# Traneptora/jxlatte

Measured on AMD Instinct MI355X. Metric: Mpixels/s decoded (VarDCT 4K frame) at 1/2/4/8 MI355X vs host-CPU jxlatte, higher is better.
Workload: dtype f32; 1 GPU; vardct4k: 8 independent 3840x2160 VarDCT frames per GPU (mix=default, Gab + EPF x2 + XYB, f32 out), inputs resident in HBM; frames_per_gpu=8, frames_total=8, frame_seeds=1000 + i, frame i on rank i mod 1, distinct_frames=8, streams=2, kernel_launches_per_frame=2

## Files before the change

jxlatte_amd/csrc/host.hip:

```cpp
#include "jxl_internal.h"
#include "modular_tend.h"
#include "pfm_check.h"
#include "varblock_check.h"
#include "palette_check.h"
#include "modchain_check.h"
#include "palette_ops.h"

#include <algorithm>
#include <chrono>
#include <cmath>
#include <cstdarg>
#include <cstdio>
#include <cstring>
#include <cstdlib>
#include <string>
#include <atomic>
#include <thread>
#include <vector>
#include <mutex>
#include <limits>

using namespace jxl;
namespace jxl {
thread_local hipEvent_t g_restore_kernel_ev[2] = {nullptr, nullptr};
// ... 172 lines not shown
    std::vector<std::pair<const jxl_ctx*, uint64_t>> batch_key;
    struct BatchLaunch { int cls, n_frames, grid_x; size_t lds_bytes, offset; };
    DevBuf batch_wg3_args;
    void* h_map16 = nullptr;
    bool map16_nofill = false;
    bool is_feeder = false;
    hipEvent_t map16_ev = nullptr;
    bool map16_inflight = false;
    hipEvent_t out_ev = nullptr;
    bool out_inflight = false;
    size_t h_map16_bytes = 0;
    bool map16_valid = false;
    DevBuf stage16;
    static constexpr int kGrpSlots = 8;
    void* h_grp = nullptr;
    const void* h_grp_dev = nullptr;
    hipEvent_t grp_ev[kGrpSlots] = {};
    bool grp_inflight[kGrpSlots] = {};
    int grp_slot = 0;
    std::vector<uint8_t> grp_written;
    uint32_t* h_sp = nullptr;
    const void* h_sp_dev = nullptr;
    size_t sp_alloc_words = 0, sp_map_words = 0;
    bool sp_valid = false;
    hipEvent_t sp_ev = nullptr;
    bool sp_inflight = false;
    SparseRec* h_sp_tab = nullptr;
    const SparseRec* h_sp_tab_dev = nullptr;
    size_t sp_tab_cap = 0, sp_tab_used = 0;
    DevBuf sp_rej;
    bool sp_rej_live = false;
    std::vector<float> h_weights_in;
    int32_t h_woffs_in[51] = {};
    DevBuf wg3_items[2];
    int wg3_item_count[2] = {0, 0};
    std::vector<BatchLaunch> batch_launches;
    hipEvent_t batch_ev = nullptr;
    bool timing = false;
    static constexpr int kEvSlots = 32;
    hipEvent_t ev[kEvSlots][3] = {};
    hipEvent_t kev[kEvSlots][2] = {};
    bool kev_valid = false;
    int ev_runs = 0;
    bool owns_stream = true;
    PlanePool* pool = nullptr;
    size_t pool_set_bytes = 0;
    size_t priv_a_bytes = 0;
    static constexpr int kAux = 12;
    int n_aux = 1;
    hipStream_t aux[kAux] = {};
    hipEvent_t fork_ev = nullptr, join_ev[kAux] = {};

    std::vector<DevBuf> mod_bufs;
    std::vector<ModOp> mod_ops;
    std::vector<ModOp> mod_ops_fused;
    std::vector<ModChan> mod_out;
    bool mod_ran = false;
    DevBuf mod_flag;
    int32_t* mod_flag_host = nullptr;
    hipEvent_t mod_ev = nullptr, mod_join = nullptr;
    bool mod_pending = false;
    int mod_redos = 0;
    int mod_launches = 0;
    std::vector<PalRun> mod_pal_runs;
    DevBuf mod_pal_count;
    unsigned int* mod_pal_count_host = nullptr;
// ... 587 lines not shown
            if (!c->hfm_sub[ch].ensure(4 * std::max<size_t>(1, h_hfm_sub[ch].size()))) return fail(c, JXL_ERR_OOM, "device allocation failed");
            HIP_TRY(c, hipMemcpyAsync(c->hfm_sub[ch].p, h_hfm_sub[ch].data(), 4 * h_hfm_sub[ch].size(), hipMemcpyHostToDevice, c->stream));
        }
        HIP_TRY(c, hipStreamSynchronize(c->stream));
    }
    const size_t nc = (size_t)c->bh * c->bw, nt = (size_t)c->th * c->tw;
    std::vector<int> wg3_tab[2];
    for (int k = 0; k < 2; k++) {
        c->wg3_item_count[k] = 0;
        for (const auto& tl : c->type_launches) {
            if (tl.cls != 2 + k) continue;
            wg3_item_table(c->h_blocks.data(), c->bw, tl.segs.data(), (int)tl.segs.size(), k, c->woffs, wg3_tab[k], wg3_grid_cap(k == 1));
            c->wg3_item_count[k] = (int)(wg3_tab[k].size() / 8);
        }
    }
    mark("item tables");
    tab_wait(c);
    {
        const volatile float cf = (float)c->p.color_factor;
        for (size_t i = 0; i < nt; i++) {
            const volatile float qx = (float)c->h_xfy[i] / cf, qb = (float)c->h_bfy[i] / cf;
            c->h_kx[i] = c->p.base_corr_x + qx;
            c->h_kb[i] = c->p.base_corr_b + qb;
        }
    }
    build_inv_sigma(c->h_hf_mul.data(), c->h_sharp.data(), nc, c->p.global_scale_f, c->p.epf_sharp_lut, c->h_isig.data());
    wg3_build_tables(c->p.quant_bias, c->p.quant_bias_numerator, c->p.scale_factor, reinterpret_cast<float*>(c->h_tab + c->off_dq));
    mark("CfL factors, inverse sigma, dequantisation tables");
    size_t o = c->tab_fixed;
    const size_t off_blocks = o, n_blk = sizeof(DevBlock) * c->h_blocks.size();
    o = tab_up(o + std::max<size_t>(16, n_blk));
    const size_t off_items = o, n_items = sizeof(WorkItem) * items.size();
    o = tab_up(o + std::max<size_t>(16, n_items));
    size_t off_wg3[2];
    for (int k = 0; k < 2; k++) {
        off_wg3[k] = o;
        o = tab_up(o + std::max<size_t>(16, sizeof(int) * wg3_tab[k].size()));
    }
    const size_t total = o;
    if (!tab_reserve(c, total, c->tab_fixed)) return fail(c, JXL_ERR_OOM, "host allocation failed (table staging)");
    tab_bind_fixed(c, nc, nt);
    if (n_blk) memcpy(c->h_tab + off_blocks, c->h_blocks.data(), n_blk);
    if (n_items) memcpy(c->h_tab + off_items, items.data(), n_items);
    for (int k = 0; k < 2; k++) {
        if (!wg3_tab[k].empty()) memcpy(c->h_tab + off_wg3[k], wg3_tab[k].data(), sizeof(int) * wg3_tab[k].size());
    }
    if (total > c->tab.cap || !c->tab.p) {
        HIP_TRY(c, hipStreamSynchronize(c->stream));
        if (!c->tab.ensure(total + total / 4)) return fail(c, JXL_ERR_OOM, "device allocation failed (frame tables)");
    }
    mark("staging");
    if (!c->tab_ev) HIP_TRY(c, hipEventCreateWithFlags(&c->tab_ev, hipEventDisableTiming));
    static const bool tab_zero = !(getenv("JXL_TABLE_ZEROCOPY") && atoi(getenv("JXL_TABLE_ZEROCOPY")) == 0);
    if (!(tab_zero && c->h_tab_pinned && copy_zero(c, c->tab.p, c->h_tab, total, false, 64, false) == 1))
        HIP_TRY(c, hipMemcpyAsync(c->tab.p, c->h_tab, total, hipMemcpyHostToDevice, c->stream));
    HIP_TRY(c, hipEventRecord(c->tab_ev, c->stream));
    c->tab_inflight = true;
    {
        char* d = static_cast<char*>(c->tab.p);
        c->hf_mul.view(d + c->off_hfm, 4 * nc);
        c->sharp.view(d + c->off_sharp, 4 * nc);
        c->xfy.view(d + c->off_kx, 4 * nt);
        c->bfy.view(d + c->off_kb, 4 * nt);
        for (int i = 0; i < 3; i++) c->lf[i].view(d + c->off_lf[i], 4 * nc);
        c->inv_sigma_tab.view(d + c->off_isig, 4 * nc);
        c->dq_tab.view(d + c->off_dq, 4 * (size_t)kWg3DqTabFloats);
        c->blocks.view(d + off_blocks, std::max<size_t>(16, n_blk));
        c->items.view(d + off_items, std::max<size_t>(16, n_items));
        for (int k = 0; k < 2; k++) c->wg3_items[k].view(d + off_wg3[k], sizeof(int) * wg3_tab[k].size());
    }
    for (const auto& job : c->lf_jobs) {
        const jxl_lfquant_desc& d = job.d;
        if (c->sub) {
            for (int ch = 0; ch < 3; ch++) {
                const int h2 = d.cells_h >> c->sy[ch], w2 = d.cells_w >> c->sx[ch], bw2 = c->bw >> c->sx[ch];
                const size_t n2 = (size_t)h2 * w2;
                if (!c->lfq_tmp[ch].ensure(4 * std::max<size_t>(1, n2))) return fail(c, JXL_ERR_OOM, "device allocation failed (LF image)");
                HIP_TRY(c, hipMemcpyAsync(c->lfq_tmp[ch].p, job.q[ch].data(), 4 * n2, hipMemcpyHostToDevice, c->stream));
                launch_lf_dequant_plain(c->lfq_tmp[ch].as<int32_t>(), c->lf[ch].as<float>(), h2, w2,
                                        (int64_t)((d.lfg_y * 256) >> c->sy[ch]) * bw2 + ((d.lfg_x * 256) >> c->sx[ch]), bw2,
                                        d.scaled_dequant[ch], d.extra_precision, c->stream);
            }
            HIP_TRY(c, hipStreamSynchronize(c->stream));
            continue;
        }
        const size_t n = (size_t)d.cells_h * d.cells_w;
        const int32_t* dq[3];
        for (int ch = 0; ch < 3; ch++) {
            if (!c->lfq_tmp[ch].ensure(4 * std::max<size_t>(1, n))) return fail(c, JXL_ERR_OOM, "device allocation failed (LF image)");
            HIP_TRY(c, hipMemcpyAsync(c->lfq_tmp[ch].p, job.q[ch].data(), 4 * n, hipMemcpyHostToDevice, c->stream));
            dq[ch] = c->lfq_tmp[ch].as<int32_t>();
        }
        float* lfp[3] = {c->lf[0].as<float>(), c->lf[1].as<float>(), c->lf[2].as<float>()};
        launch_lf_dequant(dq, lfp, d.cells_h, d.cells_w, (int64_t)(d.lfg_y * 256) * c->bw + d.lfg_x * 256, c->bw, d.scaled_dequant,
                          d.extra_precision, c->p.base_corr_x, c->p.base_corr_b, c->p.color_factor, d.x_factor_lf, d.b_factor_lf,
                          d.adaptive_smoothing, c->stream);
        HIP_TRY(c, hipStreamSynchronize(c->stream));
    }
    c->llf_alias = c->large_count == 0;
    if (!c->llf_alias)
        for (int ch = 0; ch < 3; ch++)
// ... 164 lines not shown

__global__ void k_clock_probe(unsigned long long ticks, unsigned long long* out) {
    const unsigned long long r0 = __builtin_amdgcn_s_memrealtime(), c0 = __builtin_amdgcn_s_memtime();
    unsigned long long r1 = r0;
    while (r1 - r0 < ticks) {
        __builtin_amdgcn_s_sleep(8);
        r1 = __builtin_amdgcn_s_memrealtime();
    }
    const unsigned long long c1 = __builtin_amdgcn_s_memtime();
    if (threadIdx.x == 0) {
        out[0] = c1 - c0;
        out[1] = r1 - r0;
    }
}
extern "C" int jxl_debug_wg3_item_table(const int32_t* types, const int32_t* n_blocks, int n_types, int frame_bw, int grid, int32_t* out, int cap) {
    std::vector<DevBlock> blocks;
    std::vector<IdctSegment> segs;
    int cell = 0;
    for (int k = 0; k < n_types; k++) {
        const int t = types[k];
        if (t < 0 || t >= JXL_NUM_TRANSFORM_TYPES || n_blocks[k] <= 0) return -1;
        segs.push_back(IdctSegment{t, (int)blocks.size(), n_blocks[k]});
        const int cw = JXL_TT[t].pw / 8, chh = JXL_TT[t].ph / 8;
        for (int i = 0; i < n_blocks[k]; i++, cell += cw * chh)
            blocks.push_back(DevBlock{(uint16_t)((cell / std::max(1, frame_bw)) & 0xffff), (uint16_t)(cell % std::max(1, frame_bw)), (uint32_t)t, 0u, 1});
    }
    int32_t woffs[3 * 17] = {};
    std::vector<int> tab;
    wg3_item_table(blocks.data(), frame_bw, segs.data(), (int)segs.size(), 0, woffs, tab, grid);
    const int n = (int)(tab.size() / 8);
    if (n > cap) return -1;
    std::copy(tab.begin(), tab.end(), out);
    return n;
}
extern "C" int64_t jxl_debug_intermediate_bytes(int device) {
    return device >= 0 && device < 64 ? (int64_t)g_inter_bytes[device].load(std::memory_order_relaxed) : -1;
}
extern "C" int jxl_debug_set_plane_a_tiled(int on) { return g_plane_a_tiled.exchange(on ? 1 : 0, std::memory_order_relaxed); }
extern "C" int jxl_debug_last_plane_a_tiled(const jxl_ctx* c) { return c ? c->last_plane_a_tiled : 0; }
extern "C" int jxl_debug_set_palette_fuse(int on) { return g_palette_fuse.exchange(on ? 1 : 0, std::memory_order_relaxed); }
extern "C" int jxl_debug_last_palette_run(const jxl_ctx* c, int32_t out[3]) {
    if (!c || !out) return -1;
    for (int i = 0; i < 3; i++) out[i] = c->mod_pal_stats[i];
    return 0;
}
extern "C" int jxl_debug_last_restore_launches(const jxl_ctx* c, int32_t codes[2]) {
    if (!c) return 0;
    for (int i = 0; i < 2 && codes; i++) codes[i] = i < c->last_restore_n ? c->last_restore_code[i] : 0;
    return c->last_restore_n;
}
extern "C" void jxl_debug_build_inv_sigma(const int32_t* hf_mul, const int32_t* sharpness, int64_t n, float global_scale_f,
                                          const float sharp_lut[8], float* out) {
    if (hf_mul && sharpness && sharp_lut && out && n > 0) build_inv_sigma(hf_mul, sharpness, (size_t)n, global_scale_f, sharp_lut, out);
}
extern "C" void jxl_debug_wg3_tables(const float quant_bias[3], float quant_bias_numerator, const float scale_factor[3], float* out) {
    if (quant_bias && scale_factor && out) wg3_build_tables(quant_bias, quant_bias_numerator, scale_factor, out);
}
extern "C" int64_t jxl_debug_read_inv_sigma(jxl_ctx* c, float* out, int64_t cap) {
    if (!c || !out || bind(c) != JXL_OK || !c->frame_open) return -1;
    const int64_t nc = (int64_t)c->bh * c->bw;
    if (cap < nc || finalize_tables(c) != JXL_OK || !c->inv_sigma_tab.p) return -1;
    if (hipStreamSynchronize(c->stream) != hipSuccess || hipMemcpy(out, c->inv_sigma_tab.p, 4 * (size_t)nc, hipMemcpyDeviceToHost) != hipSuccess) return -1;
    return nc;
}
extern "C" int jxl_debug_last_palette(const jxl_ctx* c, int64_t* delta_pixels) {
    if (!c) return 0;
// ... 211 lines not shown
    if (c->spl_ev) (void)hipEventDestroy(c->spl_ev);
    if (c->h_spl) {
        if (c->h_spl_pinned) (void)hipHostFree(c->h_spl);
        else free(c->h_spl);
    }
    for (auto& b : c->mod_bufs) b.release();
    for (int i = 0; i < jxl_ctx::kEvSlots; i++)
        for (int j = 0; j < 3; j++)
            if (c->ev[i][j]) (void)hipEventDestroy(c->ev[i][j]);
    for (int i = 0; i < jxl_ctx::kEvSlots; i++)
        for (int j = 0; j < 2; j++)
            if (c->kev[i][j]) (void)hipEventDestroy(c->kev[i][j]);
    if (c->fork_ev) (void)hipEventDestroy(c->fork_ev);
    if (c->batch_ev) (void)hipEventDestroy(c->batch_ev);
    c->batch_wg3_args.release();
    c->mod_flag.release();
    if (c->mod_flag_host) (void)hipHostFree(c->mod_flag_host);
    c->mod_flag_host = nullptr;
    c->mod_pal_count.release();
    if (c->mod_pal_count_host) (void)hipHostFree(c->mod_pal_count_host);
    c->mod_pal_count_host = nullptr;
    if (c->mod_ev) (void)hipEventDestroy(c->mod_ev);
    if (c->mod_join) (void)hipEventDestroy(c->mod_join);
    c->mod_ev = c->mod_join = nullptr;
    c->stage16.release();
    if (c->map16_ev) (void)hipEventDestroy(c->map16_ev);
    if (c->out_ev) (void)hipEventDestroy(c->out_ev);
    if (c->h_map16) (void)hipHostFree(c->h_map16);
    c->h_map16 = nullptr;
    if (c->sp_ev) (void)hipEventDestroy(c->sp_ev);
    if (c->h_sp) (void)hipHostFree(c->h_sp);
    if (c->h_sp_tab) (void)hipHostFree(c->h_sp_tab);
    c->sp_rej.release();
    c->wg3_items[0].release();
    c->wg3_items[1].release();
    c->batch_restore_args.release();
    for (int i = 0; i < jxl_ctx::kAux; i++) {
        if (c->aux[i]) { (void)hipStreamSynchronize(c->aux[i]); (void)hipStreamDestroy(c->aux[i]); }
        if (c->join_ev[i]) (void)hipEventDestroy(c->join_ev[i]);
    }
    if (c->stream && c->owns_stream) (void)hipStreamDestroy(c->stream);
    delete c;
}

jxl_status jxl_ctx_synchronize(jxl_ctx* c) {
    jxl_status st = bind(c);
    if (st) return st;
    HIP_TRY(c, hipStreamSynchronize(c->stream));
    return JXL_OK;
}

void* jxl_ctx_stream(jxl_ctx* c) { return c ? (void*)c->stream : nullptr; }

jxl_status jxl_ctx_set_stream(jxl_ctx* c, void* stream) {
    jxl_status st = bind(c);
    if (st) return st;
    HIP_TRY(c, hipStreamSynchronize(c->stream));
    pool_detach(c);
    if (c->owns_stream && c->stream) (void)hipStreamDestroy(c->stream);
    c->stream = (hipStream_t)stream;
    c->owns_stream = false;
    (void)pool_of(c);
    return JXL_OK;
}

jxl_status jxl_vardct_begin_frame(jxl_ctx* c, const jxl_vardct_params* p) {
// ... 798 lines not shown
    int launches = 0;
    float* B[3] = {c->planeB[0].as<float>(), c->planeB[1].as<float>(), c->planeB[2].as<float>()};
    hipEvent_t* evs = c->ev[c->ev_runs % jxl_ctx::kEvSlots];
    if (c->timing) (void)hipEventRecord(evs[0], s);
    if ((p.stages & JXL_STAGE_IDCT) && !idct_done) {
        DevFrame f;
        fill_dev_frame(c, f);
        const DevBlock* blocks = c->blocks.as<DevBlock>();
        const WorkItem* items = c->items.as<WorkItem>();
        if (c->llf_count > 0) {
            float* L[3] = {c->llf[0].as<float>(), c->llf[1].as<float>(), c->llf[2].as<float>()};
            launch_llf(f, blocks, c->llf_first, c->llf_count, L, s);
            launches++;
        }
        auto frame_of = [&](int channel) {
            DevFrame fc = f;
            if (channel >= 0) {
                fc.no_cfl = 1;
                fc.width = c->W >> c->sx[channel];
                fc.height = c->H >> c->sy[channel];
                fc.bw = c->bw >> c->sx[channel];
                fc.bh = c->bh >> c->sy[channel];
                fc.hf_mul = c->hfm_sub[channel].as<int32_t>();
            }
            return fc;
        };
        static const int wg3_grid = wg3_grid_cap(false);
        static const int wg3_grid_big = wg3_grid_cap(true);
        Wg3Args wa[2];
        int wn[2] = {0, 0};
        for (const auto& tl : c->type_launches)
            if (tl.cls >= 2) {
                const int k = tl.cls - 2;
                wn[k] = build_wg3_args(f, blocks, tl.segs.data(), (int)tl.segs.size(), k, A, wa[k], tiled);
                if (wn[k] < 0) return fail(c, JXL_ERR_STATE, "IDCT launch: too many segments");
                if (c->wg3_item_count[k] < wn[k]) return fail(c, JXL_ERR_STATE, "IDCT launch: item list out of date");
                if (wn[k] > 0) wa[k].total_items = wn[k] = c->wg3_item_count[k];
                wa[k].items = c->wg3_items[k].as<int>();
            }
        const int n_k = (int)c->type_launches.size() + (int)c->special_launches.size();
        const bool fork = n_k > 1 && c->n_aux > 0;
        if (wn[0] > 0 || wn[1] > 0) {
            hipStream_t side = fork ? c->aux[0] : s;
            if (fork) {
                (void)hipEventRecord(c->fork_ev, s);
                (void)hipStreamWaitEvent(side, c->fork_ev, 0);
            }
            if (wn[1] > 0) {
                launch_idct_wg3(wa[1], true, wg3_grid_big, side);
                launches++;
            }
            if (wn[0] > 0) {
                launch_idct_wg3(wa[0], false, wg3_grid, s);
                launches++;
            }
            if (fork) {
                (void)hipEventRecord(c->join_ev[0], side);
                (void)hipStreamWaitEvent(s, c->join_ev[0], 0);
            }
        } else {
            int used = 0;
            if (fork) {
                (void)hipEventRecord(c->fork_ev, s);
                used = std::min(n_k - 1, c->n_aux);
                for (int i = 0; i < used; i++) (void)hipStreamWaitEvent(c->aux[i], c->fork_ev, 0);
            }
            int k = 0;
// ... 182 lines not shown
        if (!c->frame_open) return fail(c, JXL_ERR_STATE, "begin_frame first");
        st = finalize_tables(c);
        if (st) return st;
        if (!ensure_private_planes(c, 4 * (size_t)c->W * c->H)) return fail(c, JXL_ERR_OOM, "device allocation failed for a %dx%d frame", c->W, c->H);
        if ((st = pre_run_zero(c))) return st;
        ok = batchable(c);
    }
    if (!ok) {
        for (int i = 0; i < n; i++) {
            const jxl_status st = run_frame(ctxs[i], false);
            if (st) return st;
        }
        return JXL_OK;
    }
    bool same = (int)c0->batch_key.size() == n;
    for (int i = 0; i < n && same; i++) same = c0->batch_key[i].first == ctxs[i] && c0->batch_key[i].second == ctxs[i]->tables_gen;
    if (!same) {
        c0->batch_launches.clear();
        std::vector<Wg3Args> wg3_args;
        for (int cls : {11, 12}) {
            const int which = cls - 11;
            jxl_ctx::BatchLaunch bl{cls, 0, 0, 0, wg3_args.size() * sizeof(Wg3Args)};
            int max_n = 0;
            for (int i = 0; i < n; i++) {
                jxl_ctx* c = ctxs[i];
                DevFrame f;
                fill_dev_frame(c, f);
                float* A[3] = {c->planeA[0].as<float>(), c->planeA[1].as<float>(), c->planeA[2].as<float>()};
                const jxl_ctx::TypeLaunch* tl = nullptr;
                for (const auto& t : c->type_launches)
                    if (t.cls == which + 2) tl = &t;
                if (!tl) continue;
                Wg3Args a;
                const int items = build_wg3_args(f, c->blocks.as<DevBlock>(), tl->segs.data(), (int)tl->segs.size(), which, A, a);
                if (items < 0) return fail(c0, JXL_ERR_STATE, "IDCT launch: too many segments");
                if (items <= 0) continue;
                if (c->wg3_item_count[which] < items) return fail(c0, JXL_ERR_STATE, "IDCT launch: item list out of date");
                a.total_items = c->wg3_item_count[which];
                a.items = c->wg3_items[which].as<int>();
                max_n = std::max(max_n, items);
                bl.lds_bytes = std::max(bl.lds_bytes, wg3_lds_bytes(a));
                wg3_args.push_back(a);
                bl.n_frames++;
            }
            if (bl.n_frames <= 0) continue;
            const int cap = wg3_grid_cap(which == 1);
            bl.grid_x = std::min(max_n, std::max(1, (cap + bl.n_frames - 1) / bl.n_frames));
            c0->batch_launches.push_back(bl);
        }
        HIP_TRY(c0, hipSetDevice(c0->device));
        if (!c0->batch_wg3_args.ensure(std::max<size_t>(sizeof(Wg3Args), wg3_args.size() * sizeof(Wg3Args))))
            return fail(c0, JXL_ERR_OOM, "device allocation failed (batch arguments)");
        HIP_TRY(c0, hipStreamSynchronize(c0->stream));
        if (c0->n_aux > 0) HIP_TRY(c0, hipStreamSynchronize(c0->aux[0]));
        if (!wg3_args.empty())
            HIP_TRY(c0, hipMemcpy(c0->batch_wg3_args.p, wg3_args.data(), wg3_args.size() * sizeof(Wg3Args), hipMemcpyHostToDevice));
        c0->batch_key.clear();
        for (int i = 0; i < n; i++) c0->batch_key.emplace_back(ctxs[i], ctxs[i]->tables_gen);
        c0->batch_restore_valid = false;
        if (!c0->batch_ev) HIP_TRY(c0, hipEventCreateWithFlags(&c0->batch_ev, hipEventDisableTiming));
    }
    hipStream_t s0 = c0->stream;
    for (int i = 1; i < n; i++) {
        (void)hipEventRecord(ctxs[i]->fork_ev, ctxs[i]->stream);
        (void)hipStreamWaitEvent(s0, ctxs[i]->fork_ev, 0);
    }
    const bool fork = c0->n_aux > 0 && c0->batch_launches.size() > 1;
// ... 2294 lines not shown
```

jxlatte_amd/csrc/jxl_internal.h:

```cpp
#pragma once
#include <hip/hip_runtime.h>
#include <vector>
#include <cmath>
#include <stdint.h>
#include "../../include/jxlatte_amd.h"
#include "../../include/jxl_transform_types.h"
#include "plane_tiled.h"
#include "blend_ops.h"
#include "patch_compile.h"
#include "modchain_check.h"

namespace jxl {

constexpr int kLutTotal = 86870;

struct DevBlock {
    uint16_t cy, cx;
    uint32_t type;
    uint32_t cfl_zero;
    int32_t hf_mul;
};

static_assert(sizeof(DevBlock) == 16, "one dwordx4 per block record");

struct WorkItem {
    uint32_t type;
    uint32_t first;
    uint32_t count;
};

struct DevFrame {
    int32_t no_cfl;
    int32_t width, height;
    int32_t bw, bh;
    int32_t tw, th;
    const int32_t* coeff[3];
    const float* lf[3];
    const float* llf[3];
    const int32_t* hf_mul;
    const int32_t* sharpness;
// ... 20 lines not shown
    for (int j = 0; j < l; j++) o += ((1 << j) - 1) << j;
    return o;
}

struct EpfParams {
    float channel_scale[3];
    float sigma_scale;
    float border_sad_mul;
    float inv_sigma_modular;
};

struct XybParams {
    float sm[9];
    float ob[3];
    float cob[3];
};

struct MultiArgs {
    static constexpr int kMaxSeg = 12;
    DevFrame f;
    const DevBlock* blocks;
    const WorkItem* items;
    int n_seg;
    int seg_b0[kMaxSeg + 1];
    int seg_n[kMaxSeg];
    int seg_type[kMaxSeg];
    int seg_first[kMaxSeg];
    int seg_nblocks[kMaxSeg];
    int nch, ch0;
    float *o0, *o1, *o2;
};
struct IdctSegment { int type, first_block, n_blocks; };

struct Wg3Seg { int type, first_block, n_blocks, item_base; };
struct Wg3Args {
    static constexpr int kMaxSeg = 21;
    DevFrame f;
    const DevBlock* blocks;
    float *o0, *o1, *o2;
    int n_seg, total_items;
    int img_floats;
    int llf_in_item;
    const int* items;
    Wg3Seg seg[kMaxSeg];
    int tiled;
};

constexpr int kWg3DqTabFloats = 3 * 128 + 3 * 256;
void wg3_build_tables(const float quant_bias[3], float quant_bias_numerator, const float scale_factor[3], float* out );
void wg3_item_table(const DevBlock* host_blocks, int frame_bw, const IdctSegment* segs, int n_seg, int which, const int32_t* woffs,
                    std::vector<int>& out, int grid);
int wg3_grid_cap(bool big);
bool wg3_handles(int type);
bool wg3_big(int type);
int build_wg3_args(const DevFrame& f, const DevBlock* blocks, const IdctSegment* segs, int n_seg, int which, float* const out[3],
                   Wg3Args& a, bool tiled = false);
void launch_idct_wg3(const Wg3Args& a, bool big, int grid_cap, hipStream_t s);
size_t wg3_lds_bytes(const Wg3Args& a);
void launch_idct_wg3_batch(const Wg3Args* dev_args, int n_frames, bool big, int grid_x, size_t lds, hipStream_t s);


int idct_class_of(int type);
void launch_idct_multi(const DevFrame& f, const DevBlock* blocks, int cls, const IdctSegment* segs, int n_seg, int ch,
                       float* const out[3], hipStream_t s);
void launch_idct_special(const DevFrame& f, const DevBlock* blocks, const WorkItem* items, int n_items, float* const out[3], hipStream_t s);
int medium_blocks_per_wg(int type);
void launch_llf(const DevFrame& f, const DevBlock* blocks, int first, int count, float* const llf[3], hipStream_t s);
void launch_idct_large(const DevFrame& f, const DevBlock* blocks, const DevBlock* host_blocks, int first, int count,
                       float* const out[3], float* const scratch[3], hipStream_t s, int* n_launches);
void launch_accumulate(int32_t* dst, const int32_t* src, int64_t n, hipStream_t s);

struct SparseRec {
    uint32_t chunk_first;
    uint32_t chunk_src;
    uint32_t count_wide;
    uint32_t where;
};
static_assert(sizeof(SparseRec) == 16, "one dwordx4 per run record");
constexpr int kSparseMaxRuns = 2048;
struct SparseGeom {
    int32_t* plane[3];
    int32_t W, H;
    int32_t sx[3], sy[3];
};
struct SparseRect { int32_t W, y0, x0, gw, gh; };
__host__ __device__ inline SparseRect sparse_rect(int W, int H, int sx, int sy, int group) {
    const int grs = (W + 255) >> 8, gy = group / grs, gx = group - gy * grs;
    const int gh = H - gy * 256 < 256 ? H - gy * 256 : 256, gw = W - gx * 256 < 256 ? W - gx * 256 : 256;
    return SparseRect{W >> sx, (gy * 256) >> sy, (gx * 256) >> sx, gw >> sx, gh >> sy};
// ... 372 lines not shown
```

jxlatte_amd/csrc/k_idct_wg3.hip:

```cpp
#include "jxl_internal.h"
#include <cstdio>
#include <cstdlib>
#include <algorithm>
#include <vector>
#include "../../include/jxl_tables.h"

namespace jxl {

#include "idct_small.h"

namespace {

#ifndef JXL_WG3_SCALAR_MAC
typedef float v2f __attribute__((ext_vector_type(2)));
__device__ __forceinline__ v2f lut_pair(const __attribute__((address_space(4))) float* lr, int j) {
    return ((const __attribute__((address_space(4))) v2f*)lr)[j];
}
#else
struct v2f {
    float x, y;
};
__device__ __forceinline__ v2f operator*(v2f a, v2f b) { return v2f{a.x * b.x, a.y * b.y}; }
__device__ __forceinline__ v2f operator+(v2f a, v2f b) { return v2f{a.x + b.x, a.y + b.y}; }
__device__ __forceinline__ v2f operator-(v2f a, v2f b) { return v2f{a.x - b.x, a.y - b.y}; }
// ... 306 lines not shown

template <int P>
__device__ __forceinline__ Item item_of(const Wg3Args& a, int& gi, int step) {
    Item it{-1, 0, 0, 0u, 0};
    while (gi < a.total_items) {
        const auto* w = (const __attribute__((address_space(4))) int*)a.items + 8 * gi;
        const int type = w[0];
        if (type != -2) {
            it.type = type;
            it.first = w[1];
            it.nb = w[2];
            it.geo = (uint32_t)w[3];
            it.gi = gi;
            break;
        }
        gi += step;
    }
    return it;
}

__device__ __forceinline__ int llf_lane_block(int tid, int lgA) { return (int)(((uint32_t)tid * 0xAAABu) >> 17) >> lgA; }

template <int NG, int WS>
struct Raw {
    v4i q[NG][3];
    v4f w[WS][3];
    float kx[NG], kb[NG];
    float hfm[NG];
    float llf;
    int rowx;
    uint32_t ok;
};

template <int NG>
struct Recs {
    int gx[NG], gz[NG], gw[NG];
    int lx;
};

template <int T, int NG>
__device__ __forceinline__ void load_recs(const Wg3Args& a, const Item& it, int tid, Recs<NG>& rc) {
    const int lgGPB = (int)((it.geo >> 4) & 15u), lgA = (int)((it.geo >> 8) & 7u);
#pragma unroll
    for (int j = 0; j < NG; j++) {
        rc.gx[j] = rc.gz[j] = 0;
        rc.gw[j] = 1;
        const int b = (tid + T * j) >> lgGPB;
        if (it.type >= 0 && b < it.nb) {
            const auto* w = (const __attribute__((address_space(4))) int*)a.blocks + 4 * (it.first + b);
            rc.gx[j] = w[0];
            rc.gz[j] = w[2];
            rc.gw[j] = w[3];
        }
    }
    rc.lx = 0;
    const int bl = llf_lane_block(tid, lgA);
    if (it.type >= 0 && bl < it.nb) rc.lx = ((const __attribute__((address_space(4))) int*)a.blocks)[4 * (it.first + bl)];
}

template <typename P>
__device__ __forceinline__ const __attribute__((address_space(1))) P* sgpr_ptr(const P* p) {
    unsigned long long u = (unsigned long long)p;
    asm volatile("" : "+s"(u));
    return (const __attribute__((address_space(1))) P*)u;
}

template <int T, int NG, int WS>
__device__ __forceinline__ void prefetch(const Wg3Args& a, const Item& it, int tid, const Recs<NG>& rc, Raw<NG, WS>& raw) {
    const DevFrame& f = a.f;
    raw.ok = 0;
    raw.llf = 0.0f;
    const int lgW4 = (int)(it.geo & 7u), lgGPB = (int)((it.geo >> 4) & 15u);
    const float* wtab = ((it.geo >> 15) & 1u) ? f.weights_t : f.weights;
    const auto* irec = (const __attribute__((address_space(4))) int*)a.items + 8 * it.gi;
    const float* wt[3] = {wtab + irec[4], wtab + irec[5], wtab + irec[6]};
    const __attribute__((address_space(1))) int32_t* cp[3] = {sgpr_ptr(f.coeff[0]), sgpr_ptr(f.coeff[1]), sgpr_ptr(f.coeff[2])};
    const auto* kxt = sgpr_ptr(f.kx_tab);
    const auto* kbt = sgpr_ptr(f.kb_tab);
    const __attribute__((address_space(1))) float* lfp[3] = {sgpr_ptr(a.llf_in_item ? f.lf[0] : f.llf[0]), sgpr_ptr(a.llf_in_item ? f.lf[1] : f.llf[1]),
                                                            sgpr_ptr(a.llf_in_item ? f.lf[2] : f.llf[2])};
    const int cells_w = f.width >> 3, tw = f.tw, bw = f.bw;
#pragma unroll
    for (int j = 0; j < NG; j++) {
        const int g = tid + T * j;
        const int b = g >> lgGPB, r = g & ((1 << lgGPB) - 1);
        const int n = r >> lgW4, x4 = (r & ((1 << lgW4) - 1)) << 2;
#pragma unroll
        for (int c = 0; c < 3; c++) {
            if (WS > 1) raw.q[j][c] = v4i{0, 0, 0, 0};
            if (WS > 1 || j == 0) raw.w[WS == 1 ? 0 : j][c] = *reinterpret_cast<const v4f*>(wt[c] + r * 4);
        }
        raw.kx[j] = raw.kb[j] = 0.0f;
        if (WS > 1) raw.hfm[j] = 1.0f;
        if (it.type >= 0 && b < it.nb && !((it.geo >> 14) & 1u)) {
            const int cy = (int)((uint32_t)rc.gx[j] & 0xffffu), cx = (int)((uint32_t)rc.gx[j] >> 16);
            const uint32_t cfl_zero = (uint32_t)rc.gz[j];
            raw.hfm[j] = (float)rc.gw[j];
            const int py = cy * 8 + n, px = cx * 8 + x4;
            const int64_t off = (((int64_t)(py >> 3) * cells_w + (px >> 3)) << 6) + (((py & 7) << 3) | (px & 7));
#pragma unroll
            for (int c = 0; c < 3; c++) raw.q[j][c] = __builtin_nontemporal_load(reinterpret_cast<const __attribute__((address_space(1))) v4i*>(cp[c] + off));
            const int ty = py >> 6, tx = px >> 6;
            const int bit = (ty - ((cy * 8) >> 6)) * 5 + (tx - ((cx * 8) >> 6));
            if (!((cfl_zero >> bit) & 1u)) {
                raw.kx[j] = kxt[ty * tw + tx];
                raw.kb[j] = kbt[ty * tw + tx];
            }
            raw.ok |= 1u << j;
        }
    }
    const int lgA = (int)((it.geo >> 8) & 7u), lgDSW = (int)((it.geo >> 12) & 3u);
    const int bl = llf_lane_block(tid, lgA);
    if (it.type >= 0 && bl < it.nb) {
        const int rr = tid - ((bl * 3) << lgA), c = rr >> lgA, k = rr & ((1 << lgA) - 1);
        const int ky = k >> lgDSW, kx = k & ((1 << lgDSW) - 1);
        const int cy = (int)((uint32_t)rc.lx & 0xffffu), cx = (int)((uint32_t)rc.lx >> 16);
        const auto* lp = c == 0 ? lfp[0] : c == 1 ? lfp[1] : lfp[2];
        raw.llf = lp[(int64_t)(cy + ky) * bw + cx + kx];
    }
    {
        constexpr int P = T * NG * 4;
        const int lgW = lgW4 + 2, lgH = lgGPB - lgW4;
        const int rb = (tid & ((P >> lgW) - 1)) >> lgH;
        raw.rowx = 0;
        if (it.type >= 0 && rb < it.nb) raw.rowx = sgpr_ptr(reinterpret_cast<const int*>(a.blocks))[4 * (it.first + rb)];
    }
}
// ... 234 lines not shown
        const int64_t off = tiled ? (int64_t)plane_tiled_off(f.width >> 3, cy * 8 + row, cx * 8) : (int64_t)(cy * 8 + row) * f.width + cx * 8;
        float* olo = out + off + (tiled ? (xlo >> 3) << 6 : xlo);
        float* ohi = out + off + (tiled ? (xhi >> 3) << 6 : xhi);
#pragma unroll
        for (int kk = 0; kk < KC / 2; kk += 4) {
            *reinterpret_cast<float4*>(olo + kk) = make_float4(acc.get(kk), acc.get(kk + 1), acc.get(kk + 2), acc.get(kk + 3));
            *reinterpret_cast<float4*>(ohi + kk) = make_float4(acc.get(KC / 2 + kk), acc.get(KC / 2 + kk + 1), acc.get(KC / 2 + kk + 2), acc.get(KC / 2 + kk + 3));
        }
    }

    static __device__ __forceinline__ void front(const Wg3Args& a, const Item& it, int tid, float* __restrict__ img, const float* __restrict__ qtab, int rowx) {
        const DevFrame& f = a.f;
        const float qbn = f.quant_bias_numerator;
        const auto* brec = (const __attribute__((address_space(4))) int*)a.blocks + 4 * it.first;
        const auto* irec = (const __attribute__((address_space(4))) int*)a.items + 8 * it.gi;
        const int cy = (int)((uint32_t)brec[0] & 0xffffu), cx = (int)((uint32_t)brec[0] >> 16);
        (void)rowx;
        const uint32_t cfl_zero = (uint32_t)brec[2];
        const int hfmul = brec[3];
        float sf[3];
        {
            const float* sft = qtab + kWg3AuxFloats;
            if ((unsigned)hfmul < (unsigned)kWg3SfEntries) {
                sf[0] = sft[hfmul];
                sf[1] = sft[kWg3SfEntries + hfmul];
                sf[2] = sft[2 * kWg3SfEntries + hfmul];
            } else {
                sf[0] = f.scale_factor[0] / (float)hfmul;
                sf[1] = f.scale_factor[1] / (float)hfmul;
                sf[2] = f.scale_factor[2] / (float)hfmul;
            }
        }
        const float* aux = qtab + kWg3QTab;
        const int cells_w = f.width >> 3, tw = f.tw;
        float dyk[16];
#pragma unroll 1
        for (int ci = 0; ci < 3; ci++) {
            const int c = ci == 0 ? 1 : ci == 1 ? 0 : 2;
            const float* wt = f.weights_t + irec[4 + c];
            const int32_t* cp = f.coeff[c];
            const float* kt = c == 0 ? f.kx_tab : f.kb_tab;
            v4i q[4];
            v4f w[4];
            float kf[4];
#pragma unroll
            for (int j = 0; j < 4; j++) {
                const int g = tid + 256 * j;
                const int n = g >> 4, x4 = (g & 15) << 2;
                const int py = cy * 8 + n, px = cx * 8 + x4;
                const int64_t off = (((int64_t)(py >> 3) * cells_w + (px >> 3)) << 6) + (((py & 7) << 3) | (px & 7));
                q[j] = __builtin_nontemporal_load(reinterpret_cast<const v4i*>(cp + off));
                w[j] = *reinterpret_cast<const v4f*>(wt + g * 4);
                kf[j] = 0.0f;
                if (c != 1) {
                    const int ty = py >> 6, tx = px >> 6;
                    const int bit = (ty - ((cy * 8) >> 6)) * 5 + (tx - ((cx * 8) >> 6));
                    if (!((cfl_zero >> bit) & 1u)) kf[j] = kt[ty * tw + tx];
                }
            }
#pragma unroll
            for (int j = 0; j < 4; j++) {
                const int g = tid + 256 * j;
                const int n = g >> 4, x4 = (g & 15) << 2;
                float dq[4];
                uint32_t big = 0;
#pragma unroll
                for (int i = 0; i < 4; i++) {
                    const uint32_t t = (uint32_t)q[j][i] + 64u;
                    big |= t;
                    dq[i] = qtab[c * 128 + (t & 127u)];
                }
                if (big >= 128u) {
#pragma unroll
                    for (int i = 0; i < 4; i++) {
// ... 89 lines not shown

}

#ifndef WG3_SMALL_OCC
#define WG3_SMALL_OCC 4
#endif
#ifndef WG3_BIG_OCC
#define WG3_BIG_OCC (WG3_BIG_T == 256 ? 2 : 4)
#endif
template <bool BIG>
__device__ __forceinline__ void wg3_body(const Wg3Args& a) {
    constexpr int P = Cls<BIG>::P, T = Cls<BIG>::T, NG = Cls<BIG>::NG, WS = Cls<BIG>::WS;
    extern __shared__ float lds[];
    const int tid0 = threadIdx.x;
    const int G = (int)gridDim.x;
#ifdef JXL_IDCT_PRIO
    __builtin_amdgcn_s_setprio(JXL_IDCT_PRIO);
#endif
    int gi = (int)blockIdx.x;
    Item cur = item_of<P>(a, gi, G);
    if (cur.type < 0) return;
    STAMP3_LIFE(0, __builtin_amdgcn_s_memtime());
    float* img = lds;
    float* qtab = lds + a.img_floats;
    const float* __restrict__ dqt = a.f.dq_tab;
    for (int i = tid0; i < kWg3QTab; i += T) qtab[i] = dqt[i];
    float* aux = qtab + kWg3QTab;
    float* lf_patch = aux + 104;
    if (tid0 < 70) aux[tid0] = a.f.lut[tid0];
    else if (tid0 >= 72 && tid0 < 104) aux[tid0] = kLlfScale3[tid0 - 72];
    for (int i = tid0; i < 3 * kWg3SfEntries; i += T)
        qtab[kWg3AuxFloats + i] = dqt[kWg3QTab + i];
    Raw<NG, WS> raw{};
    Recs<NG> rc;
    load_recs<T, NG>(a, cur, tid0, rc);
    prefetch<T, NG, WS>(a, cur, tid0, rc, raw);
    gi += G;
    Item nxt = item_of<P>(a, gi, G);
    load_recs<T, NG>(a, nxt, tid0, rc);
    auto loads_landed = [&]() {
#pragma unroll
        for (int j = 0; j < NG; j++) {
            asm volatile("" ::"v"(raw.q[j][0]), "v"(raw.q[j][1]), "v"(raw.q[j][2]), "v"(raw.kx[j]), "v"(raw.kb[j]), "v"(rc.gx[j]), "v"(rc.gz[j]),
                         "v"(rc.gw[j]));
        }
#pragma unroll
        for (int j = 0; j < WS; j++) asm volatile("" ::"v"(raw.w[j][0]), "v"(raw.w[j][1]), "v"(raw.w[j][2]));
        asm volatile("" ::"v"(raw.llf), "v"(rc.lx), "v"(raw.rowx));
    };
    loads_landed();
    if (tid0 < 192) lf_patch[tid0] = raw.llf;
    lds_barrier();
    auto landed_and_published = [&]() {
        loads_landed();
        if (tid0 < 192) lf_patch[tid0] = raw.llf;
    };
    int it_no = 0;
#pragma unroll 1
    for (;;) {
        STAMP3(0);
        int tid = tid0;
        asm volatile("" : "+v"(tid));
        do_dequant<BIG>(a, cur, tid, raw, img, qtab);
        const int rowx = raw.rowx;
        STAMP3(1);
        lds_barrier();
        STAMP3(2);
        if (!BIG && __builtin_expect(wg3_is_special(cur.type), 0)) {
            raw = Raw<NG, WS>{};
            special_phase(cur, tid);
        }
        if (!BIG && __builtin_expect(cur.type == 18, 0)) {
            raw = Raw<NG, WS>{};
            Item64::front(a, cur, tid, img, qtab, rowx);
        }
        prefetch<T, NG, WS>(a, nxt, tid, rc, raw);
        gi += G;
        const Item nn = item_of<P>(a, gi, G);
        load_recs<T, NG>(a, nn, tid, rc);
        STAMP3(3);
        do_passes<BIG>(a, cur, tid, img, it_no, rowx, landed_and_published);
        if (nxt.type < 0) break;
        cur = nxt;
        nxt = nn;
        STAMP3(9);
        lds_barrier();
        STAMP3(10);
        it_no++;
    }
    STAMP3_LIFE(1, __builtin_amdgcn_s_memtime() | ((unsigned long long)(it_no + 1) << 56));
    STAMP3_FLUSH();
}

template <bool BIG>
__global__ __launch_bounds__(Cls<BIG>::T, BIG ? WG3_BIG_OCC : WG3_SMALL_OCC) void k_idct_wg3(const Wg3Args a) {
    wg3_body<BIG>(a);
}

template <bool BIG>
__global__ __launch_bounds__(Cls<BIG>::T, BIG ? WG3_BIG_OCC : WG3_SMALL_OCC) void k_idct_wg3_batch(const Wg3Args* __restrict__ args) {
    typedef const __attribute__((address_space(4))) Wg3Args* cargs;
    wg3_body<BIG>(*(const Wg3Args*)((cargs)args + blockIdx.y));
}

#ifdef JXL_STAMPS
extern "C" int jxl_debug_set_stamps3(void* dev_ptr) {
    unsigned long long* p = (unsigned long long*)dev_ptr;
    return (int)hipMemcpyToSymbol(HIP_SYMBOL(g_stamps3), &p, sizeof p);
}
#endif

void wg3_build_tables(const float quant_bias[3], float quant_bias_numerator, const float scale_factor[3], float* out) {
// ... 2 lines not shown
        out[i] = q == 0 ? 0.0f : q == 1 ? quant_bias[c] : q == -1 ? -quant_bias[c] : (float)q - quant_bias_numerator / (float)q;
    }
    for (int i = 0; i < 3 * kWg3SfEntries; i++) {
        const int c = i / kWg3SfEntries, m = i % kWg3SfEntries;
        out[kWg3QTab + i] = scale_factor[c] / (float)(m > 0 ? m : 1);
    }
}

bool wg3_handles(int type) { return JXL_TT[type].ph < 128 && JXL_TT[type].pw < 128; }
bool wg3_big(int type) { return type == 19 || type == 20; }

int wg3_grid_cap(bool big) {
    static const int g_small = getenv("JXL_WG3_GRID") ? atoi(getenv("JXL_WG3_GRID")) : 768;
    static const int g_big = getenv("JXL_WG3_GRID_BIG") ? atoi(getenv("JXL_WG3_GRID_BIG")) : 512;
    return big ? g_big : g_small;
}

int wg3_blocks_per_item(int type) {
    const int h = JXL_TT[type].ph, w = JXL_TT[type].pw;
    if (type == 18) return 1;
    return ((h > w ? h : w) <= 32 ? 2048 : 4096) / (h * w);
}

static int wg3_img_floats(int type) {
    const int h = JXL_TT[type].ph, w = JXL_TT[type].pw;
    const int nb = wg3_blocks_per_item(type);
    if (wg3_is_special(type)) return 3 * nb * 65;
    if (type == 18) return 64 * 65;
    const int img0 = h * (w + 1);
    const int img = w >= 32 ? img0 : img0 + ((w - img0 % 32) + 32) % 32;
    return 3 * nb * img;
}

int build_wg3_args(const DevFrame& f, const DevBlock* blocks, const IdctSegment* segs, int n_seg, int which, float* const out[3],
                   Wg3Args& a, bool tiled) {
    a.f = f;
    a.blocks = blocks;
    a.o0 = out[0]; a.o1 = out[1]; a.o2 = out[2];
    a.n_seg = 0;
    a.total_items = 0;
    a.img_floats = 0;
    a.items = nullptr;
    a.llf_in_item = 1;
    a.tiled = tiled ? 1 : 0;
    static_assert(Wg3Args::kMaxSeg >= 21, "one segment per type wg3_handles() accepts");
    for (int i = 0; i < n_seg; i++) {
        if (segs[i].n_blocks <= 0 || !wg3_handles(segs[i].type) || wg3_big(segs[i].type) != (which == 1)) continue;
        if (a.n_seg >= Wg3Args::kMaxSeg) return -1;
        Wg3Seg& sg = a.seg[a.n_seg++];
        const int nb = wg3_blocks_per_item(segs[i].type);
        sg.type = segs[i].type;
        sg.first_block = segs[i].first_block;
        sg.n_blocks = segs[i].n_blocks;
        sg.item_base = a.total_items;
        a.total_items += (segs[i].n_blocks + nb - 1) / nb;
        a.img_floats = std::max(a.img_floats, wg3_img_floats(segs[i].type));
    }
    return a.total_items;
}

static float wg3_item_cost(int type) {
    switch (type) {
    case 0: return 55.f;
    case 1: case 2: case 3: case 12: case 13: case 14: case 15: case 16: case 17: return 70.f;
    case 4: return 76.f;
    case 5: return 100.f;
    case 6: case 7: return 67.f;
    case 8: case 9: return 83.f;
    case 10: case 11: return 90.f;
    case 18: return 330.f;
    default: return 100.f;
    }
}

void wg3_item_table(const DevBlock* hb, int frame_bw, const IdctSegment* segs, int n_seg, int which, const int32_t* woffs,
                    std::vector<int>& out, int grid) {
    struct Rec { uint32_t key; int type, first, nb; };
    std::vector<Rec> recs;
    constexpr int rsh = 5;
    const int grs = std::max(1, (frame_bw + (1 << rsh) - 1) >> rsh);
    for (int i = 0; i < n_seg; i++) {
        if (segs[i].n_blocks <= 0 || !wg3_handles(segs[i].type) || wg3_big(segs[i].type) != (which == 1)) continue;
        const int nb = wg3_blocks_per_item(segs[i].type);
        for (int o = 0; o < segs[i].n_blocks; o += nb) {
            const DevBlock& b0 = hb[segs[i].first_block + o];
            recs.push_back(Rec{(uint32_t)((b0.cy >> rsh) * grs + (b0.cx >> rsh)), segs[i].type, segs[i].first_block + o, std::min(nb, segs[i].n_blocks - o)});
        }
// ... 108 lines not shown
```

Before: 62010 Mpixels/s.

## Precompute per-block IDCT records with coefficient offset, CfL factors and HF multiplier

Adds a host-built 16-byte record per varblock that holds the precomputed coefficient offset, the CfL kx/kb factors for its tile, and the HF multiplier as a float. The small-class wg3 IDCT kernel now reads these records instead of decoding block coordinates and doing dependent gathers into the kx/kb tables per lane. Blocks that span several tiles or exceed the size limit are flagged and take a slow fallback path that rebuilds the values as before. The cost is extra host work and upload bandwidth per frame, plus a branchy fallback path in the prefetch code.

```diff
diff --git a/jxlatte_amd/csrc/host.hip b/jxlatte_amd/csrc/host.hip
--- a/jxlatte_amd/csrc/host.hip
+++ b/jxlatte_amd/csrc/host.hip
@@ -228,6 +228,7 @@
     bool sp_rej_live = false;
     std::vector<float> h_weights_in;
     int32_t h_woffs_in[51] = {};
+    DevBuf wg3_recs;
     DevBuf wg3_items[2];
     int wg3_item_count[2] = {0, 0};
     std::vector<BatchLaunch> batch_launches;
@@ -881,6 +882,8 @@
     o = tab_up(o + std::max<size_t>(16, n_blk));
     const size_t off_items = o, n_items = sizeof(WorkItem) * items.size();
     o = tab_up(o + std::max<size_t>(16, n_items));
+    const size_t off_recs = o, n_recs = sizeof(Wg3Block) * c->h_blocks.size();
+    o = tab_up(o + std::max<size_t>(16, n_recs));
     size_t off_wg3[2];
     for (int k = 0; k < 2; k++) {
         off_wg3[k] = o;
@@ -891,6 +894,14 @@
     tab_bind_fixed(c, nc, nt);
     if (n_blk) memcpy(c->h_tab + off_blocks, c->h_blocks.data(), n_blk);
     if (n_items) memcpy(c->h_tab + off_items, items.data(), n_items);
+    {
+        Wg3Block* hr = reinterpret_cast<Wg3Block*>(c->h_tab + off_recs);
+        const bool fit = wg3_records_fit(c->W, c->H);
+        for (size_t i = 0; i < c->h_blocks.size(); i++) {
+            const DevBlock& b = c->h_blocks[i];
+            hr[i] = wg3_block_record(b.cy, b.cx, JXL_TT[b.type].ph, JXL_TT[b.type].pw, b.cfl_zero, b.hf_mul, c->W >> 3, c->tw, c->h_kx.data(), c->h_kb.data(), fit);
+        }
+    }
     for (int k = 0; k < 2; k++) {
         if (!wg3_tab[k].empty()) memcpy(c->h_tab + off_wg3[k], wg3_tab[k].data(), sizeof(int) * wg3_tab[k].size());
     }
@@ -916,6 +927,7 @@
         c->dq_tab.view(d + c->off_dq, 4 * (size_t)kWg3DqTabFloats);
         c->blocks.view(d + off_blocks, std::max<size_t>(16, n_blk));
         c->items.view(d + off_items, std::max<size_t>(16, n_items));
+        c->wg3_recs.view(d + off_recs, std::max<size_t>(16, n_recs));
         for (int k = 0; k < 2; k++) c->wg3_items[k].view(d + off_wg3[k], sizeof(int) * wg3_tab[k].size());
     }
     for (const auto& job : c->lf_jobs) {
@@ -1146,6 +1158,20 @@
     if (n > cap) return -1;
     std::copy(tab.begin(), tab.end(), out);
     return n;
+}
+extern "C" int jxl_debug_wg3_block_records(const int32_t* blocks5, int n, int width, int height, const float* kx_tab, const float* kb_tab, uint32_t* out) {
+    if (!blocks5 || !kx_tab || !kb_tab || !out || n < 0 || width <= 0 || height <= 0 || (width & 7) || (height & 7)) return -1;
+    const int tw = (width + 63) >> 6;
+    const bool fit = wg3_records_fit(width, height);
+    for (int i = 0; i < n; i++) {
+        const int32_t* b = blocks5 + 5 * (size_t)i;
+        if (b[2] < 0 || b[2] >= JXL_NUM_TRANSFORM_TYPES) return -1;
+        const int ph = JXL_TT[b[2]].ph, pw = JXL_TT[b[2]].pw;
+        if (b[0] < 0 || b[1] < 0 || b[0] * 8 + ph > height || b[1] * 8 + pw > width) return -1;
+        const Wg3Block r = wg3_block_record(b[0], b[1], ph, pw, (uint32_t)b[3], b[4], width >> 3, tw, kx_tab, kb_tab, fit);
+        memcpy(out + 4 * (size_t)i, &r, sizeof r);
+    }
+    return 0;
 }
 extern "C" int64_t jxl_debug_intermediate_bytes(int device) {
     return device >= 0 && device < 64 ? (int64_t)g_inter_bytes[device].load(std::memory_order_relaxed) : -1;
@@ -1423,6 +1449,7 @@
     if (c->h_sp) (void)hipHostFree(c->h_sp);
     if (c->h_sp_tab) (void)hipHostFree(c->h_sp_tab);
     c->sp_rej.release();
+    c->wg3_recs.release();
     c->wg3_items[0].release();
     c->wg3_items[1].release();
     c->batch_restore_args.release();
@@ -2287,7 +2314,7 @@
         for (const auto& tl : c->type_launches)
             if (tl.cls >= 2) {
                 const int k = tl.cls - 2;
-                wn[k] = build_wg3_args(f, blocks, tl.segs.data(), (int)tl.segs.size(), k, A, wa[k], tiled);
+                wn[k] = build_wg3_args(f, blocks, c->wg3_recs.as<Wg3Block>(), tl.segs.data(), (int)tl.segs.size(), k, A, wa[k], tiled);
                 if (wn[k] < 0) return fail(c, JXL_ERR_STATE, "IDCT launch: too many segments");
                 if (c->wg3_item_count[k] < wn[k]) return fail(c, JXL_ERR_STATE, "IDCT launch: item list out of date");
                 if (wn[k] > 0) wa[k].total_items = wn[k] = c->wg3_item_count[k];
@@ -2536,7 +2563,7 @@
                     if (t.cls == which + 2) tl = &t;
                 if (!tl) continue;
                 Wg3Args a;
-                const int items = build_wg3_args(f, c->blocks.as<DevBlock>(), tl->segs.data(), (int)tl->segs.size(), which, A, a);
+                const int items = build_wg3_args(f, c->blocks.as<DevBlock>(), c->wg3_recs.as<Wg3Block>(), tl->segs.data(), (int)tl->segs.size(), which, A, a);
                 if (items < 0) return fail(c0, JXL_ERR_STATE, "IDCT launch: too many segments");
                 if (items <= 0) continue;
                 if (c->wg3_item_count[which] < items) return fail(c0, JXL_ERR_STATE, "IDCT launch: item list out of date");
diff --git a/jxlatte_amd/csrc/jxl_internal.h b/jxlatte_amd/csrc/jxl_internal.h
--- a/jxlatte_amd/csrc/jxl_internal.h
+++ b/jxlatte_amd/csrc/jxl_internal.h
@@ -6,6 +6,7 @@
 #include "../../include/jxlatte_amd.h"
 #include "../../include/jxl_transform_types.h"
 #include "plane_tiled.h"
+#include "wg3_block_record.h"
 #include "blend_ops.h"
 #include "patch_compile.h"
 #include "modchain_check.h"
@@ -92,7 +93,7 @@
 };
 struct IdctSegment { int type, first_block, n_blocks; };
 
-struct Wg3Seg { int type, first_block, n_blocks, item_base; };
+struct Wg3Seg { int type, first_block, n_blocks; };
 struct Wg3Args {
     static constexpr int kMaxSeg = 21;
     DevFrame f;
@@ -104,6 +105,7 @@
     const int* items;
     Wg3Seg seg[kMaxSeg];
     int tiled;
+    const Wg3Block* recs;
 };
 
 constexpr int kWg3DqTabFloats = 3 * 128 + 3 * 256;
@@ -113,8 +115,8 @@
 int wg3_grid_cap(bool big);
 bool wg3_handles(int type);
 bool wg3_big(int type);
-int build_wg3_args(const DevFrame& f, const DevBlock* blocks, const IdctSegment* segs, int n_seg, int which, float* const out[3],
-                   Wg3Args& a, bool tiled = false);
+int build_wg3_args(const DevFrame& f, const DevBlock* blocks, const Wg3Block* recs, const IdctSegment* segs, int n_seg, int which,
+                   float* const out[3], Wg3Args& a, bool tiled = false);
 void launch_idct_wg3(const Wg3Args& a, bool big, int grid_cap, hipStream_t s);
 size_t wg3_lds_bytes(const Wg3Args& a);
 void launch_idct_wg3_batch(const Wg3Args* dev_args, int n_frames, bool big, int grid_x, size_t lds, hipStream_t s);
diff --git a/jxlatte_amd/csrc/k_idct_wg3.hip b/jxlatte_amd/csrc/k_idct_wg3.hip
--- a/jxlatte_amd/csrc/k_idct_wg3.hip
+++ b/jxlatte_amd/csrc/k_idct_wg3.hip
@@ -362,21 +362,27 @@
     uint32_t ok;
 };
 
-template <int NG>
+template <int NG, bool REC>
 struct Recs {
     int gx[NG], gz[NG], gw[NG];
     int lx;
 };
 
-template <int T, int NG>
-__device__ __forceinline__ void load_recs(const Wg3Args& a, const Item& it, int tid, Recs<NG>& rc) {
+template <int T, int NG, bool REC>
+__device__ __forceinline__ void load_recs(const Wg3Args& a, const Item& it, int tid, Recs<NG, REC>& rc) {
     const int lgGPB = (int)((it.geo >> 4) & 15u), lgA = (int)((it.geo >> 8) & 7u);
 #pragma unroll
     for (int j = 0; j < NG; j++) {
         rc.gx[j] = rc.gz[j] = 0;
-        rc.gw[j] = 1;
+        rc.gw[j] = REC ? 0 : 1;
         const int b = (tid + T * j) >> lgGPB;
-        if (it.type >= 0 && b < it.nb) {
+        if constexpr (REC) {
+            if (it.type >= 0 && b < it.nb) {
+                const auto* w = (const __attribute__((address_space(4))) int*)a.recs + 4 * (it.first + b);
+                rc.gx[j] = w[0];
+                rc.gw[j] = w[3];
+            }
+        } else if (it.type >= 0 && b < it.nb) {
             const auto* w = (const __attribute__((address_space(4))) int*)a.blocks + 4 * (it.first + b);
             rc.gx[j] = w[0];
             rc.gz[j] = w[2];
@@ -395,8 +401,8 @@
     return (const __attribute__((address_space(1))) P*)u;
 }
 
-template <int T, int NG, int WS>
-__device__ __forceinline__ void prefetch(const Wg3Args& a, const Item& it, int tid, const Recs<NG>& rc, Raw<NG, WS>& raw) {
+template <int T, int NG, int WS, bool REC>
+__device__ __forceinline__ void prefetch(const Wg3Args& a, const Item& it, int tid, const Recs<NG, REC>& rc, Raw<NG, WS>& raw) {
     const DevFrame& f = a.f;
     raw.ok = 0;
     raw.llf = 0.0f;
@@ -405,10 +411,11 @@
     const auto* irec = (const __attribute__((address_space(4))) int*)a.items + 8 * it.gi;
     const float* wt[3] = {wtab + irec[4], wtab + irec[5], wtab + irec[6]};
     const __attribute__((address_space(1))) int32_t* cp[3] = {sgpr_ptr(f.coeff[0]), sgpr_ptr(f.coeff[1]), sgpr_ptr(f.coeff[2])};
-    const auto* kxt = sgpr_ptr(f.kx_tab);
-    const auto* kbt = sgpr_ptr(f.kb_tab);
-    const __attribute__((address_space(1))) float* lfp[3] = {sgpr_ptr(a.llf_in_item ? f.lf[0] : f.llf[0]), sgpr_ptr(a.llf_in_item ? f.lf[1] : f.llf[1]),
-                                                            sgpr_ptr(a.llf_in_item ? f.lf[2] : f.llf[2])};
+    [[maybe_unused]] const auto* kxt = REC ? nullptr : sgpr_ptr(f.kx_tab);
+    [[maybe_unused]] const auto* kbt = REC ? nullptr : sgpr_ptr(f.kb_tab);
+    const bool lii = REC || a.llf_in_item;
+    const __attribute__((address_space(1))) float* lfp[3] = {sgpr_ptr(lii ? f.lf[0] : f.llf[0]), sgpr_ptr(lii ? f.lf[1] : f.llf[1]),
+                                                            sgpr_ptr(lii ? f.lf[2] : f.llf[2])};
     const int cells_w = f.width >> 3, tw = f.tw, bw = f.bw;
 #pragma unroll
     for (int j = 0; j < NG; j++) {
@@ -422,7 +429,47 @@
         }
         raw.kx[j] = raw.kb[j] = 0.0f;
         if (WS > 1) raw.hfm[j] = 1.0f;
-        if (it.type >= 0 && b < it.nb && !((it.geo >> 14) & 1u)) {
+        if constexpr (REC) {
+            if (it.type >= 0 && b < it.nb && !((it.geo >> 14) & 1u)) {
+                const uint32_t w3 = (uint32_t)rc.gw[j];
+                const uint32_t inb = ((__umul24((uint32_t)n >> 3, (uint32_t)cells_w) + ((uint32_t)x4 >> 3)) << 6) | (uint32_t)(((n & 7) << 3) | (x4 & 7));
+                const uint32_t boff = ((uint32_t)rc.gx[j] + inb) << 2;
+#pragma unroll
+                for (int c = 0; c < 3; c++)
+                    raw.q[j][c] = __builtin_nontemporal_load(reinterpret_cast<const __attribute__((address_space(1))) v4i*>(
+                        reinterpret_cast<const __attribute__((address_space(1))) char*>(cp[c]) + boff));
+                const auto* rw = (const __attribute__((address_space(4))) float*)a.recs + 4 * (it.first + b);
+                raw.kx[j] = rw[1];
+                raw.kb[j] = rw[2];
+                raw.hfm[j] = __builtin_bit_cast(float, w3 & ~kWg3BlockFallback);
+                if (__builtin_expect(w3 & kWg3BlockFallback, 0)) {
+                    int z = 0;
+                    asm volatile("" : "+s"(z));
+                    typedef const __attribute__((address_space(1))) int* gint;
+                    typedef const __attribute__((address_space(1))) float* gfloat;
+                    const gint db = (gint)a.blocks + 4 * (it.first + b);
+                    const uint32_t d0 = (uint32_t)db[0], cfl_zero = (uint32_t)db[2];
+                    raw.hfm[j] = (float)db[3];
+                    const int cy = (int)(d0 & 0xffffu), cx = (int)(d0 >> 16);
+                    const int py = cy * 8 + n, px = cx * 8 + x4;
+                    const int fw = (&f.width)[z], fh = (&f.height)[z];
+                    if (!wg3_records_fit(fw, fh)) {
+                        const int64_t off = (((int64_t)(py >> 3) * (fw >> 3) + (px >> 3)) << 6) + (((py & 7) << 3) | (px & 7));
+#pragma unroll
+                        for (int c = 0; c < 3; c++)
+                            raw.q[j][c] = __builtin_nontemporal_load(reinterpret_cast<const __attribute__((address_space(1))) v4i*>(cp[c] + off));
+                    }
+                    const int ty = py >> 6, tx = px >> 6;
+                    const int bit = (ty - ((cy * 8) >> 6)) * 5 + (tx - ((cx * 8) >> 6));
+                    const int ti = ty * (&f.tw)[z] + tx;
+                    const bool zero = (cfl_zero >> bit) & 1u;
+                    const float tkx = ((gfloat)(&f.kx_tab)[z])[ti], tkb = ((gfloat)(&f.kb_tab)[z])[ti];
+                    raw.kx[j] = zero ? 0.0f : tkx;
+                    raw.kb[j] = zero ? 0.0f : tkb;
+                }
+                raw.ok |= 1u << j;
+            }
+        } else if (it.type >= 0 && b < it.nb && !((it.geo >> 14) & 1u)) {
             const int cy = (int)((uint32_t)rc.gx[j] & 0xffffu), cx = (int)((uint32_t)rc.gx[j] >> 16);
             const uint32_t cfl_zero = (uint32_t)rc.gz[j];
             raw.hfm[j] = (float)rc.gw[j];
@@ -723,14 +770,18 @@
             }
         }
         const float* aux = qtab + kWg3QTab;
-        const int cells_w = f.width >> 3, tw = f.tw;
+        int z = 0;
+        asm volatile("" : "+s"(z));
+        const int cells_w = f.width >> 3, tw = (&f.tw)[z];
+        const float* const kxp = (&f.kx_tab)[z];
+        const float* const kbp = (&f.kb_tab)[z];
         float dyk[16];
 #pragma unroll 1
         for (int ci = 0; ci < 3; ci++) {
             const int c = ci == 0 ? 1 : ci == 1 ? 0 : 2;
             const float* wt = f.weights_t + irec[4 + c];
             const int32_t* cp = f.coeff[c];
-            const float* kt = c == 0 ? f.kx_tab : f.kb_tab;
+            const float* kt = c == 0 ? kxp : kbp;
             v4i q[4];
             v4f w[4];
             float kf[4];
@@ -886,17 +937,21 @@
     for (int i = tid0; i < 3 * kWg3SfEntries; i += T)
         qtab[kWg3AuxFloats + i] = dqt[kWg3QTab + i];
     Raw<NG, WS> raw{};
-    Recs<NG> rc;
-    load_recs<T, NG>(a, cur, tid0, rc);
-    prefetch<T, NG, WS>(a, cur, tid0, rc, raw);
+    constexpr bool REC = !BIG;
+    Recs<NG, REC> rc;
+    load_recs<T, NG, REC>(a, cur, tid0, rc);
+    prefetch<T, NG, WS, REC>(a, cur, tid0, rc, raw);
     gi += G;
     Item nxt = item_of<P>(a, gi, G);
-    load_recs<T, NG>(a, nxt, tid0, rc);
+    load_recs<T, NG, REC>(a, nxt, tid0, rc);
     auto loads_landed = [&]() {
 #pragma unroll
         for (int j = 0; j < NG; j++) {
-            asm volatile("" ::"v"(raw.q[j][0]), "v"(raw.q[j][1]), "v"(raw.q[j][2]), "v"(raw.kx[j]), "v"(raw.kb[j]), "v"(rc.gx[j]), "v"(rc.gz[j]),
-                         "v"(rc.gw[j]));
+            if constexpr (REC)
+                asm volatile("" ::"v"(raw.q[j][0]), "v"(raw.q[j][1]), "v"(raw.q[j][2]), "v"(raw.kx[j]), "v"(raw.kb[j]), "v"(raw.hfm[j]), "v"(rc.gx[j]), "v"(rc.gw[j]));
+            else
+                asm volatile("" ::"v"(raw.q[j][0]), "v"(raw.q[j][1]), "v"(raw.q[j][2]), "v"(raw.kx[j]), "v"(raw.kb[j]), "v"(rc.gx[j]), "v"(rc.gz[j]),
+                             "v"(rc.gw[j]));
         }
 #pragma unroll
         for (int j = 0; j < WS; j++) asm volatile("" ::"v"(raw.w[j][0]), "v"(raw.w[j][1]), "v"(raw.w[j][2]));
@@ -928,10 +983,10 @@
             raw = Raw<NG, WS>{};
             Item64::front(a, cur, tid, img, qtab, rowx);
         }
-        prefetch<T, NG, WS>(a, nxt, tid, rc, raw);
+        prefetch<T, NG, WS, REC>(a, nxt, tid, rc, raw);
         gi += G;
         const Item nn = item_of<P>(a, gi, G);
-        load_recs<T, NG>(a, nn, tid, rc);
+        load_recs<T, NG, REC>(a, nn, tid, rc);
         STAMP3(3);
         do_passes<BIG>(a, cur, tid, img, it_no, rowx, landed_and_published);
         if (nxt.type < 0) break;
@@ -1000,10 +1055,11 @@
     return 3 * nb * img;
 }
 
-int build_wg3_args(const DevFrame& f, const DevBlock* blocks, const IdctSegment* segs, int n_seg, int which, float* const out[3],
-                   Wg3Args& a, bool tiled) {
+int build_wg3_args(const DevFrame& f, const DevBlock* blocks, const Wg3Block* recs, const IdctSegment* segs, int n_seg, int which,
+                   float* const out[3], Wg3Args& a, bool tiled) {
     a.f = f;
     a.blocks = blocks;
+    a.recs = recs;
     a.o0 = out[0]; a.o1 = out[1]; a.o2 = out[2];
     a.n_seg = 0;
     a.total_items = 0;
@@ -1020,7 +1076,6 @@
         sg.type = segs[i].type;
         sg.first_block = segs[i].first_block;
         sg.n_blocks = segs[i].n_blocks;
-        sg.item_base = a.total_items;
         a.total_items += (segs[i].n_blocks + nb - 1) / nb;
         a.img_floats = std::max(a.img_floats, wg3_img_floats(segs[i].type));
     }
diff --git a/jxlatte_amd/csrc/wg3_block_record.h b/jxlatte_amd/csrc/wg3_block_record.h
--- /dev/null
+++ b/jxlatte_amd/csrc/wg3_block_record.h
@@ -0,0 +1,36 @@
+#pragma once
+#include <cstdint>
+#include <cstring>
+
+namespace jxl {
+
+struct Wg3Block {
+    uint32_t off, kx, kb, hfm;
+};
+static_assert(sizeof(Wg3Block) == 16, "four dwords per block record");
+constexpr uint32_t kWg3BlockFallback = 1u;
+constexpr int64_t kWg3RecMaxSamples = (int64_t)1 << 30;
+
+constexpr bool wg3_records_fit(int width, int height) { return (int64_t)width * height <= kWg3RecMaxSamples; }
+
+inline Wg3Block wg3_block_record(int cy, int cx, int ph, int pw, uint32_t cfl_zero, int32_t hf_mul, int cells_w, int tw, const float* kx_tab,
+                                 const float* kb_tab, bool fit) {
+    Wg3Block r{0u, 0u, 0u, 0u};
+    const float hf = (float)hf_mul;
+    std::memcpy(&r.hfm, &hf, 4);
+    const int py0 = cy * 8, px0 = cx * 8;
+    const int ty0 = py0 >> 6, tx0 = px0 >> 6, ty1 = (py0 + ph - 1) >> 6, tx1 = (px0 + pw - 1) >> 6;
+    const bool one_tile = ty0 == ty1 && tx0 == tx1;
+    if ((r.hfm & kWg3BlockFallback) || !fit || !one_tile) {
+        r.hfm |= kWg3BlockFallback;
+        if (!fit) return r;
+    }
+    r.off = (uint32_t)((((int64_t)cy * cells_w) + cx) << 6);
+    if (one_tile && !(cfl_zero & 1u)) {
+        std::memcpy(&r.kx, &kx_tab[(size_t)ty0 * tw + tx0], 4);
+        std::memcpy(&r.kb, &kb_tab[(size_t)ty0 * tw + tx0], 4);
+    }
+    return r;
+}
+
+}
```

Measured after the change: 62610 Mpixels/s (median of 6 runs). No clear change (+1.0%).
